# garymm/starflate

Measured on AMD Instinct MI355X. Metric: compress MiB/s + ratio vs zlib -6, 1 GiB synthetic; 1/2/4/8 GPU, higher is better.
Workload: dtype u8; 1 GPU; 1 GiB synthetic enwik-like text per GPU (gen_text_torch seed 3); effort=default, block_bytes=524288, deflate_block_bytes=32768, window_bytes=32768, container=raw, parallelism=shard1

## Files before the change

include/starflate_hip.h:

```cpp
#ifndef STARFLATE_HIP_H
#define STARFLATE_HIP_H

#include <stddef.h>
#include <stdint.h>

#ifdef __cplusplus
extern "C" {
#endif

typedef struct sfh_ctx sfh_ctx;

enum sfh_status {
  SFH_OK = 0,
  SFH_E_INVALID_ARG = -1,
  SFH_E_DST_TOO_SMALL = -2,
  SFH_E_NO_DEVICE = -3,
  SFH_E_HIP = -4,
  SFH_E_NOMEM = -5,
  SFH_E_COMM = -6,
  SFH_E_UNSUPPORTED = -7,
  SFH_E_NOT_INDEXABLE = -8
};

enum sfh_strategy {
// ... 223 lines not shown
                             uint64_t* dst_n_out, uint32_t* status);
#define SFH_STREAM_NSTAGES 5
#define SFH_STREAM_NCOUNTS 6
int sfh_last_stream_stats(sfh_ctx* ctx, float ms[SFH_STREAM_NSTAGES], uint64_t counts[SFH_STREAM_NCOUNTS]);

size_t sfh_last_decode_scratch_bytes(const sfh_ctx* ctx);

#define SFH_INFLATE_NSTAGES 2
int sfh_last_inflate_ms(sfh_ctx* ctx, float ms[SFH_INFLATE_NSTAGES]);
const char* sfh_inflate_stage_name(int stage);


int sfh_checksum_device(sfh_ctx* ctx, const void* d_src, size_t n, uint32_t kind, uint32_t* out, void* stream);
uint32_t sfh_crc32_combine(uint32_t crc_a, uint32_t crc_b, uint64_t len_b);
uint32_t sfh_adler32_combine(uint32_t adler_a, uint32_t adler_b, uint64_t len_b);

#define SFH_NSTAGES 5

void sfh_set_profiling(sfh_ctx* ctx, int on);
int sfh_last_stage_ms(sfh_ctx* ctx, float ms[SFH_NSTAGES]);
const char* sfh_stage_name(int stage);

enum sfh_debug_what {
  SFH_DBG_NTOK = 0,
  SFH_DBG_TOKENS = 1,
  SFH_DBG_ITEMS = 8,
  SFH_DBG_NITEMS = 9,
  SFH_DBG_HIST = 2,
  SFH_DBG_PLAN = 3,
  SFH_DBG_LENS = 4,
  SFH_DBG_OFFSETS = 5,
  SFH_DBG_SUBINDEX = 7,
  SFH_DBG_SEGINFO = 10,
  SFH_DBG_STAMPS = 6
};
int sfh_debug_read(sfh_ctx* ctx, int what, void* host_dst, size_t bytes);

#ifdef __cplusplus
}
#endif
#endif
```

starflate_amd/_capi.py:

```python
import ctypes as C
import os

from . import build as _build

NSTAGES = 5
INFLATE_NSTAGES = 2
SEGMENT_BYTES = 32768
STRATEGY = {"auto": 0, "stored": 1, "fixed": 2, "dynamic": 3}
CONTAINER = {"raw": 0, "zlib": 1, "gzip": 2}
COMPRESS_CONTAINER = dict(CONTAINER, dictzip=3)
DZ_MAX_CHUNKS = 32762
E_NOT_INDEXABLE = -8
SIZE_FROM_TRAILER = (1 << 64) - 1
ITEM_NOT_INDEXABLE = 0xFFFFFFF8
DBG_NTOK, DBG_TOKENS, DBG_HIST, DBG_PLAN, DBG_LENS, DBG_OFFSETS, DBG_STAMPS = range(7)
DBG_SUBINDEX = 7
DBG_ITEMS, DBG_NITEMS = 8, 9
DBG_SEGINFO = 10
DEFAULT_BLOCK_BYTES = 262144
LARGE_BLOCK_BYTES = 1 << 19
CHAIN_BLOCK_BYTES = 1 << 20
SUBINDEX_WORDS = 64

EXPORTS = [
    "sfh_default_options", "sfh_device_count", "sfh_get_device_props", "sfh_create", "sfh_destroy", "sfh_last_error",
    "sfh_compress_bound", "sfh_compress_bound_container", "sfh_dz_header_bytes", "sfh_compress", "sfh_compress_multi", "sfh_compress_device", "sfh_compress_device_async",
    "sfh_compress_batch_device_async", "sfh_compress_batch", "sfh_batch_index_size", "sfh_copy_batch_index",
    "sfh_decompress_batch_device_async", "sfh_decompress_batch",
    "sfh_decompress_ranges_device_async", "sfh_decompress_range_device", "sfh_decompress_ranges",
    "sfh_dz_read_index", "sfh_dz_read_index_device", "sfh_decompress_dz_device", "sfh_decompress_dz", "sfh_decompress_dz_ranges",
    "sfh_bgzf_bound", "sfh_compress_bgzf_device_async", "sfh_compress_bgzf_device", "sfh_compress_bgzf",
    "sfh_bgzf_read_index", "sfh_bgzf_read_index_device", "sfh_decompress_bgzf_device", "sfh_decompress_bgzf",
    "sfh_decompress_bgzf_wide_device",
    "sfh_decompress_bgzf_ranges_device", "sfh_decompress_bgzf_ranges", "sfh_bgzf_voffsets_to_offsets", "sfh_bgzf_offsets_to_voffsets",
    "sfh_zip_read_index", "sfh_zip_read_index_device", "sfh_decompress_zip_device", "sfh_decompress_zip", "sfh_zip_bound",
    "sfh_compress_zip_device_async", "sfh_compress_zip_device", "sfh_compress_zip",
    "sfh_recover_index_device", "sfh_recover_index", "sfh_decompress_any_device", "sfh_decompress_any", "sfh_last_recover_stats",
    "sfh_recover_index_batch_device", "sfh_recover_index_batch", "sfh_decompress_any_batch_device", "sfh_decompress_any_batch",
    "sfh_inflate_stream_device", "sfh_inflate_stream", "sfh_inflate_stream_batch_device", "sfh_inflate_stream_batch",
    "sfh_last_stream_stats",
    "sfh_last_block_bytes", "sfh_index_entries", "sfh_copy_index", "sfh_copy_subindex", "sfh_decompress_device", "sfh_decompress", "sfh_last_inflate_ms", "sfh_last_decode_scratch_bytes",
    "sfh_inflate_stage_name", "sfh_checksum_device", "sfh_crc32_combine", "sfh_adler32_combine",
    "sfh_set_profiling", "sfh_last_stage_ms", "sfh_stage_name", "sfh_debug_read",
    "sfh_gather_offsets", "sfh_gather_streams", "sfh_comm_ranks", "sfh_lds_order_check",
]


class Options(C.Structure):
    _fields_ = [("strategy", C.c_uint32), ("final_stream", C.c_uint32), ("lazy", C.c_uint32),
                ("no_stored_fast_path", C.c_uint32), ("container", C.c_uint32), ("block_bytes", C.c_uint32),
                ("effort", C.c_uint32), ("chain_depth", C.c_uint32)]
# ... 267 lines not shown
```

starflate_amd/compressor.py:

```python
import ctypes as C

import numpy as np

from . import _capi

CHUNK_BYTES = 32768
ITEM_NOT_INDEXABLE = _capi.ITEM_NOT_INDEXABLE


class StarflateError(RuntimeError):
    def __init__(self, code, msg):
        super().__init__(f"starflate_hip error {code}: {msg}")
        self.code = code


class Compressor:

    def __init__(self, device=0):
        self._lib = _capi.lib()
        n = self._lib.sfh_device_count()
        if n <= 0:
            raise StarflateError(-3, "no HIP device visible; the compressor has no CPU fallback")
        h = C.c_void_p()
        rc = self._lib.sfh_create(C.byref(h), int(device))
# ... 818 lines not shown

        if not (isinstance(t, torch.Tensor) and t.is_cuda and t.dtype == torch.uint8 and t.dim() == 1 and t.is_contiguous()):
            raise ValueError("expected a contiguous 1-D uint8 CUDA tensor")
        if t.device.index != self.device:
            raise ValueError(f"tensor is on cuda:{t.device.index}, compressor on cuda:{self.device}")

    def lds_order_check(self, op, blocks=256, iters=50):
        bad, n = C.c_uint64(0), C.c_uint64(0)
        rc = self._lib.sfh_lds_order_check(self._h, int(op), int(blocks), int(iters), C.byref(bad), C.byref(n))
        if rc:
            raise StarflateError(rc, self._lib.sfh_last_error(self._h).decode())
        return bad.value, n.value

    def set_profiling(self, on=True):
        self._lib.sfh_set_profiling(self._h, int(bool(on)))

    def stage_ms(self):
        ms = (C.c_float * _capi.NSTAGES)()
        self._check(self._lib.sfh_last_stage_ms(self._h, C.byref(ms)))
        return {self._lib.sfh_stage_name(k).decode(): float(ms[k]) for k in range(_capi.NSTAGES)}

    def debug(self, what, nchunks):
        shapes = {
            _capi.DBG_NTOK: ((nchunks,), np.uint32),
            _capi.DBG_TOKENS: ((nchunks, CHUNK_BYTES), np.uint32),
            _capi.DBG_HIST: ((nchunks, 576), np.uint32),
            _capi.DBG_PLAN: ((nchunks, 4), np.uint32),
            _capi.DBG_LENS: ((nchunks, 320), np.uint8),
            _capi.DBG_OFFSETS: ((nchunks,), np.uint64),
            _capi.DBG_STAMPS: ((2, nchunks, 8), np.uint64),
            _capi.DBG_SUBINDEX: ((nchunks, 32, 2), np.uint32),
            _capi.DBG_ITEMS: ((nchunks, CHUNK_BYTES), np.uint16),
            _capi.DBG_NITEMS: ((nchunks,), np.uint32),
            _capi.DBG_SEGINFO: ((nchunks, 6), np.uint32),
        }
        shape, dt = shapes[what]
        a = np.empty(shape, dtype=dt)
        self._check(self._lib.sfh_debug_read(self._h, what, a.ctypes.data, a.nbytes))
        return a

    def debug_tokens(self, nchunks):
        items = self.debug(_capi.DBG_ITEMS, nchunks)
        nit = self.debug(_capi.DBG_NITEMS, nchunks)
        toks, flags = [], []
        for c in range(nchunks):
            if nit[c] & 0x80000000:
                raise StarflateError(-1, f"chunk {c} took the stored fast path: its items are not materialised (stored_fast_path=False shows them)")
            it = items[c, : nit[c]].astype(np.uint32)
            start = (it & 0x8000) != 0
            head = start & ((it & 0x0100) != 0)
            assert not np.any(head[:-1] & start[1:]) and (it.size == 0 or not head[-1]), "a head without its distance"
            nxt = np.zeros(it.size, dtype=np.uint32)
            nxt[:-1] = it[1:]
            tok = np.where(head, np.uint32(0x80000000) | ((it & 0xFF) << 16) | (nxt & 0x7FFF), it & 0xFF)[start]
            fl = ((it & 0x4000) != 0)[start]
            reg = ((it >> 9) & 31)[start]
            toks.append(tok.astype(np.uint32))
            flags.append([(int(k), int(reg[k])) for k in np.flatnonzero(fl)])
        return toks, flags


def compress_multi(compressors, data, strategy="auto", final_stream=True, lazy=True, stored_fast_path=True, container="raw",
                   block_bytes=0):
    L = _capi.lib()
    src = np.frombuffer(data, dtype=np.uint8) if not isinstance(data, np.ndarray) else np.ascontiguousarray(data, dtype=np.uint8)
    cap = L.sfh_compress_bound(src.size, 0)
# ... 417 lines not shown
```

starflate_amd/csrc/sf_capi.hip:

```cpp
#include "../../include/starflate_hip.h"
#include "sf_any_plan.h"
#include "sf_bgzf_plan.h"
#include "sf_bgzf_range_plan.h"
#include "sf_device.h"
#include "sf_dz_plan.h"
#include "sf_inflate_core.h"
#include "sf_inflate_plan.h"
#include "sf_range_plan.h"
#include "sf_scratch.h"
#include "sf_stage_plan.h"
#include "sf_zip_plan.h"

#include <dlfcn.h>
#include <stdio.h>
#include <stdlib.h>
#include <string.h>
#include <algorithm>
#include <memory>
#include <new>
#include <thread>
#include <vector>

namespace {
using sf::scratch::Buf;
// ... 3444 lines not shown
int sfh_last_stage_ms(sfh_ctx* ctx, float ms[SFH_NSTAGES]) {
  if (!ctx || !ms || !ctx->ev_valid) return SFH_E_INVALID_ARG;
  for (int k = 0; k < SFH_NSTAGES; ++k) ms[k] = 0.f;
  for (uint32_t b = 0; b < ctx->ev_batches; ++b) {
    const Event* e = &ctx->ev[(size_t)b * sfh_ctx::kEvPerBatch];
    for (int k = 0; k < 4; ++k) {
      float t = 0.f;
      SF_HIP(hipEventElapsedTime(&t, e[k], e[k + 1]), "elapsed");
      ms[k] += t;
    }
  }
  const size_t last = (size_t)ctx->ev_batches * sfh_ctx::kEvPerBatch;
  SF_HIP(hipEventElapsedTime(&ms[4], ctx->ev[last - 1], ctx->ev[last]), "elapsed");
  return SFH_OK;
}

const char* sfh_stage_name(int stage) {
  static const char* names[SFH_NSTAGES] = {"k_lz77", "k_plan", "k_scan", "k_emit", "k_checksum"};
  return (stage >= 0 && stage < SFH_NSTAGES) ? names[stage] : "";
}

int sfh_debug_read(sfh_ctx* ctx, int what, void* host_dst, size_t bytes) {
  if (!ctx || !host_dst || !ctx->last_chunks) return SFH_E_INVALID_ARG;
  const size_t nlast = std::min<size_t>(ctx->last_chunks, std::max<uint32_t>(ctx->batch_chunks, sf::kMaxStrip / sf::kChunk));
  const size_t nc = std::min<size_t>(nlast, ctx->cap_batch), nidx = std::min<size_t>(ctx->last_chunks, ctx->cap_chunks);
  if (int rc = wait_idle(ctx)) return rc;
  const void* p = nullptr;
  size_t avail = 0;
  switch (what) {
    case SFH_DBG_NTOK: p = ctx->ws.ntok; avail = nc * 4; break;
    case SFH_DBG_TOKENS: p = ctx->ws.tokens; avail = ctx->cap_dtok >= nlast ? nlast * sf::kChunk * 4 : 0; break;
    case SFH_DBG_ITEMS: p = ctx->ws.items; avail = nc * sf::kChunk * 2; break;
    case SFH_DBG_NITEMS: p = ctx->ws.nitems; avail = nc * 4; break;
    case SFH_DBG_HIST: p = ctx->ws.hist; avail = nc * sf::kHistStride * 4; break;
    case SFH_DBG_PLAN: p = ctx->ws.plan; avail = nc * sizeof(sf::ChunkPlan); break;
    case SFH_DBG_OFFSETS: p = ctx->ws.offsets; avail = nidx * 8; break;
    case SFH_DBG_SUBINDEX: p = ctx->ws.subidx; avail = nidx * SFH_SUBINDEX_WORDS * 4; break;
    case SFH_DBG_STAMPS: p = ctx->ws.stamps; avail = p ? nc * 128 : 0; break;
    case SFH_DBG_SEGINFO: p = ctx->ws.seginfo; avail = std::min<size_t>(ctx->last_chunks * sizeof(sf::SegInfo), ctx->seginfo_cap); break;
    case SFH_DBG_LENS: {
      if (!ctx->ws.codes || bytes > nc * 320) return SFH_E_INVALID_ARG;
      SF_HIP(hipSetDevice(ctx->device), "hipSetDevice");
      SF_HIP(hipMemcpy2D(host_dst, 320, (const uint8_t*)ctx->ws.codes + offsetof(sf::ChunkCodes, lens),
                         sizeof(sf::ChunkCodes), 320, bytes / 320, hipMemcpyDeviceToHost), "debug copy");
      return SFH_OK;
    }
    default: return SFH_E_INVALID_ARG;
  }
  if (!p || bytes > avail) return SFH_E_INVALID_ARG;
  SF_HIP(hipSetDevice(ctx->device), "hipSetDevice");
  SF_HIP(hipMemcpy(host_dst, p, bytes, hipMemcpyDeviceToHost), "debug copy");
  return SFH_OK;
}

}
```

starflate_amd/csrc/sf_device.h:

```cpp
#pragma once
#include <hip/hip_runtime.h>
#include <stdint.h>

#include <vector>

#include "sf_stream_chain.h"

namespace sf {

constexpr uint32_t kChunk = 32768;
constexpr uint32_t kWindow = 32768;
constexpr uint32_t kWideRow = 65536;
constexpr uint32_t kStep = 1024;
constexpr uint32_t kHashBits = 13;
constexpr uint32_t kMaxStrip = 1u << 24;
constexpr uint32_t kRegion = 512;
constexpr uint32_t kSubBytes = 1024;
constexpr uint32_t kCap = 16;
constexpr uint32_t kMinMatch = 4;
constexpr uint32_t kFar4 = 4096;
constexpr uint32_t kSkipSlack = 128;
constexpr uint32_t kSkipProbe = 2048;
constexpr uint32_t kItemsSkipped = 0x80000000u;
constexpr uint32_t kSubRegions = kChunk / kSubBytes;
constexpr uint32_t kTokMatch = 0x80000000u;
constexpr uint32_t kTokRegion = 0x40000000u;
constexpr uint32_t kItemTok = 0x8000u;
constexpr uint32_t kItemRegion = 0x4000u;
constexpr uint32_t kItemRegionShift = 9;
constexpr uint32_t kItemHead = 0x0100u;

constexpr uint32_t kChecksumAdler32 = 1;
constexpr uint32_t kChecksumCrc32 = 2;
constexpr uint32_t kCrcPoly = 0xEDB88320u;

constexpr uint32_t kHistStride = 576;
constexpr uint32_t kHistD = 288;
constexpr uint32_t kHistLen = 320;
constexpr uint32_t kHeaderWords = 152;

template <int CTRL, int ROW_MASK>
__device__ __forceinline__ uint32_t dpp_from(uint32_t v) {
  return (uint32_t)__builtin_amdgcn_update_dpp(0, (int)v, CTRL, ROW_MASK, 0xF, false);
}
template <int CTRL, int ROW_MASK>
__device__ __forceinline__ uint32_t dpp_add_from(uint32_t v) {
  return v + (uint32_t)__builtin_amdgcn_update_dpp(0, (int)v, CTRL, ROW_MASK, 0xF, false);
}
__device__ __forceinline__ uint32_t wave_incl_add(uint32_t v) {
  v = dpp_add_from<0x111, 0xF>(v);
  v = dpp_add_from<0x112, 0xF>(v);
  v = dpp_add_from<0x114, 0xF>(v);
  v = dpp_add_from<0x118, 0xF>(v);
  v = dpp_add_from<0x142, 0xA>(v);
  v = dpp_add_from<0x143, 0xC>(v);
  return v;
}
__device__ __forceinline__ uint32_t wave_excl_max(uint32_t v) {
  v = max(v, dpp_from<0x111, 0xF>(v));
  v = max(v, dpp_from<0x112, 0xF>(v));
  v = max(v, dpp_from<0x114, 0xF>(v));
  v = max(v, dpp_from<0x118, 0xF>(v));
  v = max(v, dpp_from<0x142, 0xA>(v));
// ... 364 lines not shown
```

starflate_amd/csrc/sf_kernels.hip:

```cpp
#include "sf_device.h"

#include <stdlib.h>

namespace sf {

__device__ __forceinline__ uint32_t len_symbol(uint32_t l3, uint32_t& ebits, uint32_t& eval) {
  if (l3 == 255) { ebits = 0; eval = 0; return 285; }
  if (l3 < 8) { ebits = 0; eval = 0; return 257 + l3; }
  const uint32_t e = (31 - __builtin_clz(l3)) - 2;
  ebits = e;
  eval = l3 & ((1u << e) - 1);
  return 257 + 4 * e + 4 + ((l3 >> e) & 3);
}
__device__ __forceinline__ uint32_t dist_symbol(uint32_t d1, uint32_t& ebits, uint32_t& eval) {
  if (d1 < 4) { ebits = 0; eval = 0; return d1; }
  const uint32_t hb = 31 - __builtin_clz(d1);
  const uint32_t e = hb - 1;
  ebits = e;
  eval = d1 & ((1u << e) - 1);
  return 2 * hb + ((d1 >> e) & 1);
}
__device__ __forceinline__ uint32_t dist_symbol_of(uint32_t d1) {
  const uint32_t x = d1 > 2u ? d1 : 2u;
  const uint32_t hb = 31 - __builtin_clz(x);
// ... 920 lines not shown
            else walk(ne);
          }
        }
      }
      stamp(3);
      static_assert(kWindow == 4 * kRound && 8 * K1_THREADS == kRound && kLook % 8 == 0, "shift: four pieces per thread and the look-ahead");
      [[maybe_unused]] uint2 sh_0 = make_uint2(0, 0), sh_1 = sh_0, sh_2 = sh_0, B_early = sh_0;
      if constexpr (EARLY) {
        asm volatile("" ::: "memory");
        const uint2* s2 = reinterpret_cast<const uint2*>(smem + L_DATA);
        sh_0 = s2[kRound / 8 + t];
        sh_1 = s2[2 * kRound / 8 + t];
        sh_2 = s2[3 * kRound / 8 + t];
        B_early = s2[kWindow / 8 + t];
      }
      const uint32_t cm = marks & T;
      const uint32_t mine = (uint32_t)__popc(marks) | ((uint32_t)__popc(cm) << 16);
      const uint32_t incl = wave_incl_add(mine);
      if (lane == 63) s_wtot[wave] = incl;
      if constexpr (EARLY)
        asm volatile("" : "+v"(sh_0.x), "+v"(sh_0.y), "+v"(sh_1.x), "+v"(sh_1.y), "+v"(sh_2.x), "+v"(sh_2.y),
                          "+v"(B_early.x), "+v"(B_early.y));
      __syncthreads();
      uint32_t wbase, rtotal;
      {
        const uint32_t w = lane < K1_WAVES ? s_wtot[lane] : 0u;
        const uint32_t wi = wave_incl_add(w);
        rtotal = (uint32_t)__builtin_amdgcn_readlane((int)wi, K1_WAVES - 1);
        wbase = (uint32_t)__builtin_amdgcn_readlane((int)(wi - w), (int)wave);
      }
      static_assert(kSkipSpan == kRound, "the probe span is the chunk's first round");
      const bool skip_now = rc == 0 && fast_skip && (n - cstart) > kSkipSpan && (rtotal & 0xFFFFu) >= kSkipSpan - kSkipSlack;
      if (!skip_now && (wave & (kSubBytes / kRegion - 1)) == 0 && lane == 0)
        rtok_out[chunk * kSubRegions + rc * kRSubs + wave / (kSubBytes / kRegion)] = tot_tok + (wbase & 0xFFFFu);
      stamp(4);
      __builtin_amdgcn_s_setprio(0);

      if constexpr (EARLY) {
        if (!skip_now && r + 1 < nrounds) {
          uint2* s2 = reinterpret_cast<uint2*>(smem + L_DATA);
          s2[t] = sh_0;
          s2[kRound / 8 + t] = sh_1;
          s2[2 * kRound / 8 + t] = sh_2;
          s2[3 * kRound / 8 + t] = B_early;
          if (t >= K1_THREADS - kLook / 8) s2[kWindow / 8 + t - (K1_THREADS - kLook / 8)] = s2[(kWindow + kRound) / 8 + t - (K1_THREADS - kLook / 8)];
          *reinterpret_cast<uint2*>(&s_data[(kWindow + kLook) / 4 + 2 * t]) = make_uint2(pre_lo, pre_hi);
          age(rb + kRound);
          staged = true;
        }
      }
      if (__builtin_expect(skip_now, 0)) {
        const uint32_t clen = (n - cstart) < kChunk ? (n - cstart) : kChunk;
        const uint2 B = EARLY ? B_early : *reinterpret_cast<const uint2*>(&s_bytes[kWindow + 8 * t]);
        bool pstore = false;
        if (clen == kChunk) {
          static_assert(256 * 32 * 4 <= kWindow && kWindow / 16 == 2 * K1_THREADS, "the copies fill the window");
          static_assert(kRoundsPerChunk == 4, "the fast path's loads");
          uint4* const z4 = reinterpret_cast<uint4*>(smem + L_DATA);
          z4[t] = make_uint4(0, 0, 0, 0);
          z4[K1_THREADS + t] = make_uint4(0, 0, 0, 0);
          __syncthreads();
          uint32_t* const rep = s_data + (lane & 31u);
          auto count8 = [&](uint32_t lo, uint32_t hi) {
#pragma unroll
            for (uint32_t j = 0; j < 8; ++j) atomicAdd(&rep[(((j < 4 ? lo : hi) >> (8 * (j & 3))) & 0xFFu) * 32u], 1u);
          };
          auto fold = [&]() -> uint32_t {
// ... 10 lines not shown
            uint32_t e = ((t & 3u) == 0 && f) ? f * (est_log2(kSkipSpan) - est_log2(f)) : 0u;
            e = wave_sum(e);
            if (lane == 0) s_wtot[wave] = e;
            __syncthreads();
            const uint32_t ent = (uint32_t)__builtin_amdgcn_readfirstlane((int)wave_sum(lane < K1_WAVES ? s_wtot[lane] : 0u));
            pstore = ((ent >> 8) + 7) / 8 + kStoreMargin >= kSkipSpan;
          }
          if (!pstore) {
            uint2 w[kRoundsPerChunk - 1];
            w[0] = make_uint2(pre_lo, pre_hi);
            w[1] = *reinterpret_cast<const uint2*>(sp + cstart + 2 * kRound + kLook + 8 * t);
            w[2] = make_uint2(0, 0);
            const bool tail = 8 * t + kLook < kRound;
            if (tail) w[2] = *reinterpret_cast<const uint2*>(sp + cstart + 3 * kRound + kLook + 8 * t);
            const uint32_t look = t < kLook / 4 ? s_data[(kWindow + kRound) / 4 + t] : 0u;
            count8(w[0].x, w[0].y);
            count8(w[1].x, w[1].y);
            if (tail) count8(w[2].x, w[2].y);
            if (t < kLook / 4) {
#pragma unroll
              for (uint32_t j = 0; j < 4; ++j) atomicAdd(&rep[((look >> (8 * j)) & 0xFFu) * 32u], 1u);
            }
            __syncthreads();
            const uint32_t sum = fold();
            if ((t & 3u) == 0) s_hist[t >> 2] = sum;
          }
        } else {
#pragma unroll
          for (uint32_t k = 0; k < 8; ++k) atomicAdd(&s_hist[((k < 4 ? B.x : B.y) >> (8 * (k & 3))) & 0xFFu], 1u);
          for (uint32_t pos = cstart + kRound + t; pos < cstart + clen; pos += K1_THREADS) atomicAdd(&s_hist[sp[pos]], 1u);
        }
        const uint32_t r_last = (r + kRoundsPerChunk - 1 < nrounds ? r + kRoundsPerChunk - 1 : nrounds - 1);
        const uint32_t ctok = pstore ? 0u : clen;
        if (t < kSubRegions) rtok_out[chunk * kSubRegions + t] = t * kSubBytes < ctok ? t * kSubBytes : ctok;
        skip = true;
        lds_stale = true;
        stale_span = short_probe ? kSkipProbe : kSkipSpan;
        chunk_done = true;
        tot_tok = ctok;
        tot_items = ctok;
        rtotal = 0;
        r = r_last;
      } else
      if (marks) {
        const uint32_t before = wbase + incl - mine;
        const uint32_t ib0 = 2u * (tot_items + (before & 0xFFFFu) + (before >> 16));
        const uint32_t both = marks | (cm << 8);
        auto item_at = [&](uint32_t below) { return ib0 + 2u * (uint32_t)__popc(both & (below | (below << 8))); };
        const uint2 B = EARLY ? B_early : *reinterpret_cast<const uint2*>(&s_bytes[kWindow + pb]);
        uint32_t t_now = t;
        asm volatile("" : "+v"(t_now));
        const uint32_t flag = (t_now & (kSubBytes / 8 - 1)) == 0 ? (kItemRegion | ((rc * kRSubs + (8 * t_now) / kSubBytes) << kItemRegionShift)) : 0u;
        auto put_item = [&](uint32_t byte_off, uint32_t v) {
          *reinterpret_cast<uint16_t*>(reinterpret_cast<uint8_t*>(gi) + (uint64_t)byte_off) = (uint16_t)v;
        };
        const uint32_t lits = marks & ~cm;
#pragma unroll
        for (uint32_t k = 0; k < 8; ++k) {
          if ((lits >> k) & 1) {
            const uint32_t b = ((k < 4 ? B.x : B.y) >> (8 * (k & 3))) & 0xFFu;
            put_item(item_at((1u << k) - 1u), k == 0 ? (kItemTok | b | flag) : (kItemTok | b));
            atomicAdd(&s_hist[b], 1u);
          }
        }
        static_assert(kMinMatch >= 4, "at most two matches start in eight positions");
        uint32_t rest = cm;
#pragma unroll
        for (uint32_t it = 0; it < 2; ++it) {
          if (rest) {
            const uint32_t k = (uint32_t)__builtin_ctz(rest);
            rest &= rest - 1u;
            const uint32_t at = item_at((1u << k) - 1u);
            uint32_t l3 = (N >> (4 * k)) & 15u;
            uint32_t d1 = dm1_of(k);
            if (l3 == kCap - 3) {
              l3 = cap_len - 3;
              d1 = cap_run ? 0u : d1;
            }
            put_item(at, (kItemTok | kItemHead | l3) | (k == 0 ? flag : 0u));
            put_item(at + 2, d1);
            atomicAdd(&s_hist[kHistLen + l3], 1u);
            atomicAdd(&s_hist[kHistD + smem[LD + (d1 < 256 ? d1 : 256 + (d1 >> 7))]], 1u);
          }
        }
      }
      tot_tok += rtotal & 0xFFFFu;
      tot_items += (rtotal & 0xFFFFu) + (rtotal >> 16);
      if constexpr (STAMPS) __syncthreads();
      stamp(5);
    }

    if (chunk_done || rc == kRoundsPerChunk - 1 || r + 1 == nrounds) {
      __syncthreads();
      if (!(chunk_done && tot_tok == 0))
        for (uint32_t idx = t; idx < kHistStride; idx += K1_THREADS) {
          hist_out[(uint64_t)chunk * kHistStride + idx] = s_hist[idx];
          s_hist[idx] = (idx == 256) ? 1u : 0u;
        }
      if (t == 0) { ntok_out[chunk] = tot_tok; nitems_out[chunk] = tot_items | (skip ? kItemsSkipped : 0u); }
      const uint32_t covered = chunk_done ? kSubRegions : (rc + 1) * kRSubs;
      if (t < kSubRegions && t >= covered) rtok_out[chunk * kSubRegions + t] = tot_tok;
      stamp(6);
    }
  }
  if (nrounds == 0) {
    for (uint32_t idx = t; idx < kHistStride; idx += K1_THREADS) hist_out[(uint64_t)chunk0 * kHistStride + idx] = (idx == 256) ? 1u : 0u;
    if (t == 0) { ntok_out[chunk0] = 0; nitems_out[chunk0] = 0; }
    if (t < kSubRegions) rtok_out[chunk0 * kSubRegions + t] = 0;
  }
  if constexpr (STAMPS) {
    if (t == 0)
      for (int k = 0; k < 8; ++k) stamps[(uint64_t)strip * 8 + k] = st_acc[k];
  }
}


__device__ __forceinline__ void or_bits(uint32_t* stage, uint32_t bitpos, uint64_t value) {
  const uint32_t w = bitpos >> 5, sh = bitpos & 31;
  const uint64_t v0 = value << sh;
  const uint32_t v2 = sh ? (uint32_t)(value >> (64 - sh)) : 0u;
  const uint32_t lo = (uint32_t)v0, mid = (uint32_t)(v0 >> 32);
  if (lo) atomicOr(&stage[w], lo);
  if (mid) atomicOr(&stage[w + 1], mid);
  if (v2) atomicOr(&stage[w + 2], v2);
}

struct PlanSmem {
  uint32_t freq[320];
  uint32_t key[288];
  union {
    uint16_t w[576];
    struct { uint16_t w_head[64]; uint8_t rle_sym[320]; uint8_t rle_ext[320]; };
  };
  union {
// ... 630 lines not shown
  if (t == 0) {
    const uint64_t all = base + s_tile[K3_TILES];
    if constexpr (!BATCH) *total = all;
    offsets[nchunks] = all + lead;
  }
  if constexpr (BATCH) {
    __syncthreads();
    for (uint32_t i = t; i < nitems; i += K3_THREADS) {
      BatchItem& I = bitems[i];
      const uint64_t g0 = offsets[I.chunk0], g1 = offsets[I.chunk0 + I.nchunks];
      const uint64_t start = I.carry ? total[I.out] : hdr;
      I.shift = start - g0;
      total[I.out] = start + (g1 - g0);
    }
  }
}

constexpr uint32_t K4_THREADS = 512;
constexpr uint32_t K4_WAVES = K4_THREADS / 64;
constexpr uint32_t K4_IPT = 8;
constexpr uint32_t K4_STAGE_FORCED = 9392;
constexpr uint32_t K4_STAGE_AUTO = 8200;
static_assert(4 * K4_STAGE_FORCED >= 3 + kChunk + kChunk / 8 + 640 + 16 + 8, "k_emit: the stage holds the largest chunk");
static_assert(4 * K4_STAGE_AUTO >= 3 + kChunk + kStoredExtra - 1 + 16 + 8, "k_emit: the small stage holds the largest chunk "
              "plan_chunk codes under strategy 0");
static_assert(K4_STAGE_FORCED % 4 == 0 && K4_STAGE_AUTO % 4 == 0, "the stage is zeroed in 16-byte steps");
template <uint32_t STAGE_WORDS>
struct EmitLds {
  alignas(16) uint32_t stage[STAGE_WORDS];
  uint32_t lcode[288];
  uint32_t dcode[32];
  uint32_t tab[1024];
  uint32_t wtot[2][K4_WAVES];
  uint32_t rtok[kSubRegions];
};
template <uint32_t STAGE_WORDS>
constexpr uint32_t k4_waves_per_simd() { return STAGE_WORDS == K4_STAGE_AUTO ? 8 : 6; }
static_assert(k4_waves_per_simd<K4_STAGE_AUTO>() / 2 * sizeof(EmitLds<K4_STAGE_AUTO>) <= 160 * 1024, "k_emit: four workgroups per CU");
static_assert(k4_waves_per_simd<K4_STAGE_FORCED>() / 2 * sizeof(EmitLds<K4_STAGE_FORCED>) <= 160 * 1024, "k_emit: three workgroups per CU");

typedef uint16_t u16x2 __attribute__((ext_vector_type(2)));
typedef int16_t s16x2 __attribute__((ext_vector_type(2)));

__device__ __forceinline__ void literal_bits(uint32_t byte, const uint32_t* lcode, uint64_t& value, uint32_t& nb) {
  const uint32_t lc = lcode[byte];
  value = lc & 0xFFFF;
  nb = lc >> 16;
}
__device__ __forceinline__ uint32_t lenlut_entry(uint32_t l3, const uint32_t* lcode) {
  uint32_t le, lv;
  const uint32_t lc = lcode[len_symbol(l3, le, lv)];
  const uint32_t p = lc >> 16;
  return (lc & 0xFFFFu) | (lv << p) | ((p + le) << 24);
}
__device__ __forceinline__ void match_bits(uint32_t l3, uint32_t d1, const uint32_t* lenlut, const uint32_t* dcode,
                                           uint64_t& value, uint32_t& nb) {
  uint32_t de, dv;
  const uint32_t ds = dist_symbol(d1, de, dv);
  const uint32_t le = lenlut[l3], dc = dcode[ds];
  uint32_t p = le >> 24;
  uint64_t v = le & 0xFFFFFFu;
  v |= (uint64_t)(dc & 0xFFFF) << p;
  p += dc >> 16;
  v |= (uint64_t)dv << p;
  p += de;
  value = v;
  nb = p;
}

template <bool BATCH, uint32_t STAGE_WORDS>
__global__ __launch_bounds__(K4_THREADS, k4_waves_per_simd<STAGE_WORDS>()) void k_emit(const uint8_t* __restrict__ src, uint64_t n_total,
                                                     uint32_t , uint16_t* items,
                                                     const uint32_t* __restrict__ nitems_in,
                                                     const uint32_t* __restrict__ ntok_in,
                                                     const ChunkPlan* __restrict__ plan,
                                                     const ChunkCodes* __restrict__ codes,
                                                     const uint64_t* __restrict__ offsets,
                                                     const uint32_t* __restrict__ rtok,
                                                     uint32_t* __restrict__ subidx,
                                                     uint8_t* __restrict__ dst_all,
                                                     const BatchChunk* __restrict__ bchunks,
                                                     const BatchItem* __restrict__ bitems) {
  __shared__ EmitLds<STAGE_WORDS> L;
  uint32_t(&s_stage)[STAGE_WORDS] = L.stage;
  uint32_t(&s_lcode)[288] = L.lcode;
  uint32_t(&s_dcode)[32] = L.dcode;
  uint32_t(&s_tab)[1024] = L.tab;
  uint32_t(&s_wtot)[2][K4_WAVES] = L.wtot;
  uint32_t(&s_rtok)[kSubRegions] = L.rtok;
  static_assert(K4_THREADS == 512, "one table entry per thread and kind");
  constexpr uint32_t kTabLit = 512, kTabLen = 768, kTabDistN = 510;

  const uint32_t t = threadIdx.x, lane = t & 63;
  const uint32_t wave = (uint32_t)__builtin_amdgcn_readfirstlane((int)(t >> 6));
  const uint32_t chunk = blockIdx.x;
  const ChunkPlan P = plan[chunk];
  const uint8_t* csrc;
  uint8_t* dst;
  uint64_t off = offsets[chunk];
  uint32_t n_raw;
  if constexpr (BATCH) {
    const BatchChunk B = bchunks[chunk];
    const BatchItem& I = bitems[B.item >> 1];
    csrc = B.src;
    n_raw = B.n_raw;
    dst = I.dst;
    off += I.shift;
  } else {
    const uint64_t cbase = (uint64_t)chunk * kChunk;
    csrc = src + cbase;
    n_raw = (uint32_t)((n_total - cbase) < (uint64_t)kChunk ? (n_total - cbase) : kChunk);
    dst = dst_all;
  }
  const ChunkCodes& C = codes[chunk];
  uint32_t pre_code = t < 288 ? C.lcode[t] : (t < 320 ? C.dcode[t - 288] : 0u);
  uint32_t pre_rtok = t < kSubRegions ? rtok[(uint64_t)chunk * kSubRegions + t] : 0u;
  const uint32_t pre_ntok = ntok_in[chunk], pre_nit = nitems_in[chunk];
  asm volatile("" : "+v"(pre_code), "+v"(pre_rtok));

  uint32_t* const sub = subidx + (uint64_t)chunk * 2 * kSubRegions;
  if (P.btype == 0) {
    if (t < 2 * kSubRegions) sub[t] = 0;
// ... 38 lines not shown
    }
    const uint32_t head = (uint32_t)((4 - ((uintptr_t)d & 3)) & 3);
    const uint32_t h = head < n_raw ? head : n_raw;
    if (t < h) d[t] = sp[t];
    const uint32_t nd = (n_raw - h) / 4;
    uint32_t* d32 = reinterpret_cast<uint32_t*>(d + h);
    const uint32_t* s32 = reinterpret_cast<const uint32_t*>(sp);
    const uint32_t full_src_words = n_raw / 4;
    for (uint32_t k = t; k < nd; k += K4_THREADS) {
      const uint32_t ob = h + 4 * k;
      const uint32_t w = ob >> 2;
      uint32_t lo = s32[w], hi = 0;
      if ((ob & 3) != 0) {
        if (w + 1 < full_src_words) hi = s32[w + 1];
        else
          for (uint32_t b = 0; b < 4 && 4 * (w + 1) + b < n_raw; ++b) hi |= (uint32_t)sp[4 * (w + 1) + b] << (8 * b);
      }
      d32[k] = __builtin_amdgcn_alignbyte(hi, lo, ob & 3);
    }
    const uint32_t done = h + 4 * nd;
    if (t < n_raw - done) d[done + t] = sp[done + t];
    return;
  }

  const uint32_t sh = (uint32_t)(off & 3);
  const uint32_t nwords = (sh + P.out_bytes + 3) / 4;
  {
    uint4* z = reinterpret_cast<uint4*>(s_stage);
    for (uint32_t k = t; k < (nwords + 2 + 3) / 4 && k < STAGE_WORDS / 4; k += K4_THREADS) z[k] = make_uint4(0, 0, 0, 0);
  }
  if (t < 288) s_lcode[t] = pre_code;
  else if (t < 320) s_dcode[t - 288] = pre_code;
  if (t < kSubRegions) {
    s_rtok[t] = pre_rtok;
    sub[2 * t + 1] = pre_rtok;
  }
  __syncthreads();
  if (t < 256) {
    const uint32_t le = lenlut_entry(t, s_lcode);
    s_tab[kTabLen + t] = (le & 0xFFFFFu) | (le >> 24) * (1u << 20 | 1u << 27);
    s_tab[kTabLit + t] = (pre_code & 0xFFFFu) | (pre_code >> 16) * (1u << 20 | 1u << 27);
  }
  if (t < kTabDistN) {
    const uint32_t sym = dist_symbol_of(t < 256 ? t : (t - 254) << 7);
    const uint32_t dc = s_dcode[sym];
    s_tab[t] = (dc & 0xFFFFu) | ((dc >> 16) << 20) | (((dc >> 16) + dist_extra_of_sym(sym)) << 27);
  } else {
    s_tab[t] = 0;
  }
  {
    uint8_t* sb = reinterpret_cast<uint8_t*>(s_stage) + sh;
    const uint8_t* hb = reinterpret_cast<const uint8_t*>(C.header);
    const uint32_t hbytes = (P.header_bits + 7) / 8;
    for (uint32_t k = t; k < hbytes; k += K4_THREADS) sb[k] = hb[k];
  }
  __syncthreads();

  const uint32_t ntok = pre_ntok;
  const uint32_t nit = pre_nit & ~kItemsSkipped;
  const uint16_t* it = items + (uint64_t)chunk * kChunk;
  if (pre_nit & kItemsSkipped) {
    uint16_t* const wr = items + (uint64_t)chunk * kChunk;
    for (uint32_t pos = t; pos < nit; pos += K4_THREADS) {
      const uint32_t b = csrc[pos];
      wr[pos] = (uint16_t)(kItemTok | ((pos & (kSubBytes - 1)) == 0 ? (b | kItemRegion | ((pos / kSubBytes) << kItemRegionShift)) : b));
    }
    __threadfence_block();
    __syncthreads();
  }
  uint32_t running = 8 * sh + P.header_bits;
  uint32_t buf = 0;
  uint4 q_next = make_uint4(0, 0, 0, 0);
  if (nit) q_next = *reinterpret_cast<const uint4*>(it + t * K4_IPT);
  for (uint32_t b0 = 0; b0 < nit; b0 += K4_THREADS * K4_IPT, buf ^= 1) {
    const uint32_t i0 = b0 + t * K4_IPT;
    const uint4 q = q_next;
    const bool full = b0 + K4_THREADS * K4_IPT <= nit;
    if (b0 + K4_THREADS * K4_IPT < nit) q_next = *reinterpret_cast<const uint4*>(it + i0 + K4_THREADS * K4_IPT);
    const uint32_t qd[K4_IPT / 2] = {q.x, q.y, q.z, q.w};
    uint32_t val[K4_IPT], nb[K4_IPT], mine = 0;
    uint32_t ent[K4_IPT];
#pragma unroll
    for (uint32_t j = 0; j < K4_IPT / 2; ++j) {
      static_assert(kItemHead == 0x100 && kTabLen == kTabLit + 0x100 && kTabLit == 0x200, "a token's low nine bits are its table index");
      static_assert(kItemTok == 0x8000, "bit 15 tells a token's first item from a distance");
      const u16x2 w = __builtin_bit_cast(u16x2, qd[j]);
      const uint32_t itok = (qd[j] & 0x01FF01FFu) | (kTabLit * 0x10001u);
      const u16x2 idist = __builtin_elementwise_min(w, (u16x2)(w >> (uint16_t)7) + (uint16_t)254);
      uint32_t tok = __builtin_bit_cast(uint32_t, __builtin_bit_cast(s16x2, w) >> (int16_t)15);
      asm volatile("" : "+v"(tok));
      const uint32_t idx = (tok & itok) | (~tok & __builtin_bit_cast(uint32_t, idist));
      const uint32_t by = __builtin_bit_cast(uint32_t, (u16x2)(__builtin_bit_cast(u16x2, idx) << (uint16_t)2));
      ent[2 * j] = *reinterpret_cast<const uint32_t*>(reinterpret_cast<const uint8_t*>(s_tab) + (by & 0xFFFFu));
      ent[2 * j + 1] = *reinterpret_cast<const uint32_t*>(reinterpret_cast<const uint8_t*>(s_tab) + (by >> 16));
    }
    asm volatile("" : "+v"(ent[0]), "+v"(ent[1]), "+v"(ent[2]), "+v"(ent[3]), "+v"(ent[4]), "+v"(ent[5]), "+v"(ent[6]), "+v"(ent[7]));
    auto both = [](uint32_t w) { return w & (w << 1) & 0x80008000u; };
    auto sbit = [](uint32_t k) { return (k & 1) ? 15 + k : k; };
    uint32_t starts = (both(q.x) >> 15) | (both(q.y) >> 13) | (both(q.z) >> 11) | (both(q.w) >> 9);
    if (!full) {
      uint32_t left = nit - i0;
      left = i0 < nit ? left : 0u;
#pragma unroll
      for (uint32_t k = 0; k < K4_IPT; ++k) {
        ent[k] = k < left ? ent[k] : 0u;
        starts &= k < left ? ~0u : ~(1u << sbit(k));
      }
    }
    const uint32_t s0 = starts ? (uint32_t)__builtin_ctz(starts) : 32u;
    const bool walk = __ballot((starts & (starts - 1)) != 0) != 0;
    uint32_t off0 = 0;
#pragma unroll
    for (uint32_t k = 0; k < K4_IPT; ++k) {
      const uint32_t en = ent[k];
      const uint32_t dl = en >> 20, n = en >> 27;
      val[k] = (__builtin_amdgcn_ubfe(qd[k / 2], 16 * (k & 1), (n - dl) & 31u) << (dl & 31u)) | (en & 0xFFFFFu);
      nb[k] = n;
      asm volatile("" : "+v"(val[k]), "+v"(nb[k]));
      off0 = s0 == sbit(k) ? mine : off0;
      mine += nb[k];
    }
    uint32_t region0;
    {
      const uint32_t j = (s0 >> 1) & 3u;
      const uint32_t w = j == 0 ? q.x : j == 1 ? q.y : j == 2 ? q.z : q.w;
      region0 = (w >> ((s0 & 16u) + kItemRegionShift)) & 31u;
    }
    const uint32_t incl = wave_incl_add(mine);
    if (lane == 63) s_wtot[buf][wave] = incl;
    __syncthreads();
    uint32_t pre = 0, all = 0;
#pragma unroll
    for (uint32_t w = 0; w < K4_WAVES; ++w) {
      const uint32_t v = s_wtot[buf][w];
      if (w < wave) pre += v;
      all += v;
    }
    const uint32_t pos = running + pre + incl - mine;
    if (walk) {
      const uint4 r = *reinterpret_cast<const uint4*>(it + i0);
      const uint32_t rd[K4_IPT / 2] = {r.x, r.y, r.z, r.w};
      uint32_t pk = pos;
#pragma unroll
      for (uint32_t k = 0; k < K4_IPT; ++k) {
        const uint32_t e = (rd[k / 2] >> (16 * (k & 1))) & 0xFFFFu;
        if ((e & (kItemTok | kItemRegion)) == (kItemTok | kItemRegion) && i0 + k < nit)
          sub[2 * ((e >> kItemRegionShift) & 31u)] = pk - 8 * sh;
        pk += nb[k];
      }
    } else if (starts) {
      sub[2 * region0] = pos + off0 - 8 * sh;
    }
    uint32_t wi = pos >> 5, ab = pos & 31;
    uint64_t acc = 0;
    auto put = [&](uint32_t v32, uint32_t n) {
      acc |= (uint64_t)v32 << ab;
      ab += n;
      if (ab >= 32) {
        atomicOr(&s_stage[wi++], (uint32_t)acc);
        acc >>= 32;
        ab -= 32;
      }
    };
#pragma unroll
    for (uint32_t k = 0; k < K4_IPT; ++k) put(val[k], nb[k]);
    if (ab) atomicOr(&s_stage[wi], (uint32_t)acc);
    running += all;
  }
  __syncthreads();
  if (t < kSubRegions && s_rtok[t] >= ntok) sub[2 * t] = running - 8 * sh;
  if (t == 0) {
    const uint32_t eob = s_lcode[256];
    or_bits(s_stage, running, eob & 0xFFFF);
    const uint32_t endbit = running + (eob >> 16);
    if (!(C.header[0] & 1u)) {
      const uint32_t byte = (endbit + 3 + 7) / 8;
      or_bits(s_stage, 8 * (byte + 2), 0xFFFFull);
    }
  }
  __syncthreads();

  uint8_t* gbase = dst + (off - sh);
  uint32_t* g32 = reinterpret_cast<uint32_t*>(gbase);
  const uint32_t lo_b = sh, hi_b = sh + P.out_bytes;
  for (uint32_t w = t; w < nwords; w += K4_THREADS) {
    const uint32_t v = s_stage[w];
    if (4 * w >= lo_b && 4 * w + 4 <= hi_b) {
      g32[w] = v;
    } else {
#pragma unroll
      for (uint32_t b = 0; b < 4; ++b) {
        const uint32_t idx = 4 * w + b;
        if (idx >= lo_b && idx < hi_b) gbase[idx] = (uint8_t)(v >> (8 * b));
      }
    }
  }
}

hipError_t init_kernels() { return hipSuccess; }

hipError_t launch_lz77(const uint8_t* src, uint64_t n, uint32_t nchunks, const Workspace& ws,
                       const Options& opt, hipStream_t s, const BatchTables* bt) {
  if (opt.strip_bytes == 0 || opt.strip_bytes % kChunk || opt.strip_bytes > kMaxStrip) return hipErrorInvalidValue;
// ... 80 lines not shown
```

Baseline: 238,800 MiB/s.

## Record per-region item index in rtok to locate subindex starts in encoder

```diff
diff --git a/include/starflate_hip.h b/include/starflate_hip.h
--- a/include/starflate_hip.h
+++ b/include/starflate_hip.h
@@ -279,6 +279,7 @@
   SFH_DBG_OFFSETS = 5,
   SFH_DBG_SUBINDEX = 7,
   SFH_DBG_SEGINFO = 10,
+  SFH_DBG_RITEM = 11,
   SFH_DBG_STAMPS = 6
 };
 int sfh_debug_read(sfh_ctx* ctx, int what, void* host_dst, size_t bytes);
diff --git a/starflate_amd/_capi.py b/starflate_amd/_capi.py
--- a/starflate_amd/_capi.py
+++ b/starflate_amd/_capi.py
@@ -17,6 +17,7 @@
 DBG_SUBINDEX = 7
 DBG_ITEMS, DBG_NITEMS = 8, 9
 DBG_SEGINFO = 10
+DBG_RITEM = 11
 DEFAULT_BLOCK_BYTES = 262144
 LARGE_BLOCK_BYTES = 1 << 19
 CHAIN_BLOCK_BYTES = 1 << 20
diff --git a/starflate_amd/compressor.py b/starflate_amd/compressor.py
--- a/starflate_amd/compressor.py
+++ b/starflate_amd/compressor.py
@@ -874,6 +874,7 @@
             _capi.DBG_SUBINDEX: ((nchunks, 32, 2), np.uint32),
             _capi.DBG_ITEMS: ((nchunks, CHUNK_BYTES), np.uint16),
             _capi.DBG_NITEMS: ((nchunks,), np.uint32),
+            _capi.DBG_RITEM: ((nchunks, 32), np.uint32),
             _capi.DBG_SEGINFO: ((nchunks, 6), np.uint32),
         }
         shape, dt = shapes[what]
diff --git a/starflate_amd/csrc/sf_capi.hip b/starflate_amd/csrc/sf_capi.hip
--- a/starflate_amd/csrc/sf_capi.hip
+++ b/starflate_amd/csrc/sf_capi.hip
@@ -3500,6 +3500,13 @@
     case SFH_DBG_TOKENS: p = ctx->ws.tokens; avail = ctx->cap_dtok >= nlast ? nlast * sf::kChunk * 4 : 0; break;
     case SFH_DBG_ITEMS: p = ctx->ws.items; avail = nc * sf::kChunk * 2; break;
     case SFH_DBG_NITEMS: p = ctx->ws.nitems; avail = nc * 4; break;
+    case SFH_DBG_RITEM: {
+      if (!ctx->ws.rtok || bytes % 4 || bytes > nc * sf::kSubRegions * 4) return SFH_E_INVALID_ARG;
+      SF_HIP(hipSetDevice(ctx->device), "hipSetDevice");
+      SF_HIP(hipMemcpy(host_dst, ctx->ws.rtok, bytes, hipMemcpyDeviceToHost), "debug copy");
+      for (size_t k = 0; k < bytes / 4; ++k) static_cast<uint32_t*>(host_dst)[k] >>= 16;
+      return SFH_OK;
+    }
     case SFH_DBG_HIST: p = ctx->ws.hist; avail = nc * sf::kHistStride * 4; break;
     case SFH_DBG_PLAN: p = ctx->ws.plan; avail = nc * sizeof(sf::ChunkPlan); break;
     case SFH_DBG_OFFSETS: p = ctx->ws.offsets; avail = nidx * 8; break;
diff --git a/starflate_amd/csrc/sf_device.h b/starflate_amd/csrc/sf_device.h
--- a/starflate_amd/csrc/sf_device.h
+++ b/starflate_amd/csrc/sf_device.h
@@ -29,6 +29,8 @@
 constexpr uint32_t kItemRegion = 0x4000u;
 constexpr uint32_t kItemRegionShift = 9;
 constexpr uint32_t kItemHead = 0x0100u;
+static_assert(kChunk <= 0x8000u, "a chunk's token and item counts fit 16 bits each");
+constexpr uint32_t region_word(uint32_t tokens_before, uint32_t items_before) { return tokens_before | (items_before << 16); }
 
 constexpr uint32_t kChecksumAdler32 = 1;
 constexpr uint32_t kChecksumCrc32 = 2;
diff --git a/starflate_amd/csrc/sf_kernels.hip b/starflate_amd/csrc/sf_kernels.hip
--- a/starflate_amd/csrc/sf_kernels.hip
+++ b/starflate_amd/csrc/sf_kernels.hip
@@ -976,7 +976,8 @@
       static_assert(kSkipSpan == kRound, "the probe span is the chunk's first round");
       const bool skip_now = rc == 0 && fast_skip && (n - cstart) > kSkipSpan && (rtotal & 0xFFFFu) >= kSkipSpan - kSkipSlack;
       if (!skip_now && (wave & (kSubBytes / kRegion - 1)) == 0 && lane == 0)
-        rtok_out[chunk * kSubRegions + rc * kRSubs + wave / (kSubBytes / kRegion)] = tot_tok + (wbase & 0xFFFFu);
+        rtok_out[chunk * kSubRegions + rc * kRSubs + wave / (kSubBytes / kRegion)] =
+            region_word(tot_tok + (wbase & 0xFFFFu), tot_items + (wbase & 0xFFFFu) + (wbase >> 16));
       stamp(4);
       __builtin_amdgcn_s_setprio(0);
 
@@ -1053,7 +1054,10 @@
         }
         const uint32_t r_last = (r + kRoundsPerChunk - 1 < nrounds ? r + kRoundsPerChunk - 1 : nrounds - 1);
         const uint32_t ctok = pstore ? 0u : clen;
-        if (t < kSubRegions) rtok_out[chunk * kSubRegions + t] = t * kSubBytes < ctok ? t * kSubBytes : ctok;
+        if (t < kSubRegions) {
+          const uint32_t before = t * kSubBytes < ctok ? t * kSubBytes : ctok;
+          rtok_out[chunk * kSubRegions + t] = region_word(before, before);
+        }
         skip = true;
         lds_stale = true;
         stale_span = short_probe ? kSkipProbe : kSkipSpan;
@@ -1120,7 +1124,7 @@
         }
       if (t == 0) { ntok_out[chunk] = tot_tok; nitems_out[chunk] = tot_items | (skip ? kItemsSkipped : 0u); }
       const uint32_t covered = chunk_done ? kSubRegions : (rc + 1) * kRSubs;
-      if (t < kSubRegions && t >= covered) rtok_out[chunk * kSubRegions + t] = tot_tok;
+      if (t < kSubRegions && t >= covered) rtok_out[chunk * kSubRegions + t] = region_word(tot_tok, tot_items);
       stamp(6);
     }
   }
@@ -1817,7 +1821,7 @@
   uint32_t dcode[32];
   uint32_t tab[1024];
   uint32_t wtot[2][K4_WAVES];
-  uint32_t rtok[kSubRegions];
+  uint32_t rtab[2 * kSubRegions];
 };
 template <uint32_t STAGE_WORDS>
 constexpr uint32_t k4_waves_per_simd() { return STAGE_WORDS == K4_STAGE_AUTO ? 8 : 6; }
@@ -1872,7 +1876,7 @@
   uint32_t(&s_dcode)[32] = L.dcode;
   uint32_t(&s_tab)[1024] = L.tab;
   uint32_t(&s_wtot)[2][K4_WAVES] = L.wtot;
-  uint32_t(&s_rtok)[kSubRegions] = L.rtok;
+  uint32_t(&s_rtab)[2 * kSubRegions] = L.rtab;
   static_assert(K4_THREADS == 512, "one table entry per thread and kind");
   constexpr uint32_t kTabLit = 512, kTabLen = 768, kTabDistN = 510;
 
@@ -1977,8 +1981,9 @@
   if (t < 288) s_lcode[t] = pre_code;
   else if (t < 320) s_dcode[t - 288] = pre_code;
   if (t < kSubRegions) {
-    s_rtok[t] = pre_rtok;
-    sub[2 * t + 1] = pre_rtok;
+    s_rtab[t] = pre_rtok & 0xFFFFu;
+    s_rtab[kSubRegions + t] = pre_rtok >> 16;
+    sub[2 * t + 1] = pre_rtok & 0xFFFFu;
   }
   __syncthreads();
   if (t < 256) {
@@ -2040,21 +2045,12 @@
       ent[2 * j + 1] = *reinterpret_cast<const uint32_t*>(reinterpret_cast<const uint8_t*>(s_tab) + (by >> 16));
     }
     asm volatile("" : "+v"(ent[0]), "+v"(ent[1]), "+v"(ent[2]), "+v"(ent[3]), "+v"(ent[4]), "+v"(ent[5]), "+v"(ent[6]), "+v"(ent[7]));
-    auto both = [](uint32_t w) { return w & (w << 1) & 0x80008000u; };
-    auto sbit = [](uint32_t k) { return (k & 1) ? 15 + k : k; };
-    uint32_t starts = (both(q.x) >> 15) | (both(q.y) >> 13) | (both(q.z) >> 11) | (both(q.w) >> 9);
     if (!full) {
       uint32_t left = nit - i0;
       left = i0 < nit ? left : 0u;
 #pragma unroll
-      for (uint32_t k = 0; k < K4_IPT; ++k) {
-        ent[k] = k < left ? ent[k] : 0u;
-        starts &= k < left ? ~0u : ~(1u << sbit(k));
-      }
-    }
-    const uint32_t s0 = starts ? (uint32_t)__builtin_ctz(starts) : 32u;
-    const bool walk = __ballot((starts & (starts - 1)) != 0) != 0;
-    uint32_t off0 = 0;
+      for (uint32_t k = 0; k < K4_IPT; ++k) ent[k] = k < left ? ent[k] : 0u;
+    }
 #pragma unroll
     for (uint32_t k = 0; k < K4_IPT; ++k) {
       const uint32_t en = ent[k];
@@ -2062,14 +2058,7 @@
       val[k] = (__builtin_amdgcn_ubfe(qd[k / 2], 16 * (k & 1), (n - dl) & 31u) << (dl & 31u)) | (en & 0xFFFFFu);
       nb[k] = n;
       asm volatile("" : "+v"(val[k]), "+v"(nb[k]));
-      off0 = s0 == sbit(k) ? mine : off0;
       mine += nb[k];
-    }
-    uint32_t region0;
-    {
-      const uint32_t j = (s0 >> 1) & 3u;
-      const uint32_t w = j == 0 ? q.x : j == 1 ? q.y : j == 2 ? q.z : q.w;
-      region0 = (w >> ((s0 & 16u) + kItemRegionShift)) & 31u;
     }
     const uint32_t incl = wave_incl_add(mine);
     if (lane == 63) s_wtot[buf][wave] = incl;
@@ -2082,38 +2071,54 @@
       all += v;
     }
     const uint32_t pos = running + pre + incl - mine;
-    if (walk) {
-      const uint4 r = *reinterpret_cast<const uint4*>(it + i0);
-      const uint32_t rd[K4_IPT / 2] = {r.x, r.y, r.z, r.w};
-      uint32_t pk = pos;
-#pragma unroll
-      for (uint32_t k = 0; k < K4_IPT; ++k) {
-        const uint32_t e = (rd[k / 2] >> (16 * (k & 1))) & 0xFFFFu;
-        if ((e & (kItemTok | kItemRegion)) == (kItemTok | kItemRegion) && i0 + k < nit)
-          sub[2 * ((e >> kItemRegionShift) & 31u)] = pk - 8 * sh;
-        pk += nb[k];
-      }
-    } else if (starts) {
-      sub[2 * region0] = pos + off0 - 8 * sh;
-    }
-    uint32_t wi = pos >> 5, ab = pos & 31;
-    uint64_t acc = 0;
+    const uint32_t wi0 = b0 + wave * (64 * K4_IPT);
+    const uint32_t rit = s_rtab[kSubRegions + (lane & (kSubRegions - 1))];
+    const bool mine_due = rit - wi0 < 64 * K4_IPT && rit < nit;
+    uint32_t due = (uint32_t)__ballot(mine_due);
+    if (__builtin_popcount(due) > 2) {
+      uint32_t a = nb[0] | nb[1] << 8 | nb[2] << 16 | nb[3] << 24, b = nb[4] | nb[5] << 8 | nb[6] << 16;
+      a += a << 8;
+      a += a << 16;
+      b += b << 8;
+      b += b << 16;
+      b += (a >> 24) * 0x010101u;
+      const uint32_t at = rit - wi0, from = ((at / K4_IPT) & 63u) * 4, slot = at & (K4_IPT - 1);
+      const uint32_t pos_o = (uint32_t)__builtin_amdgcn_ds_bpermute((int)from, (int)pos);
+      const uint32_t a_o = (uint32_t)__builtin_amdgcn_ds_bpermute((int)from, (int)a);
+      const uint32_t b_o = (uint32_t)__builtin_amdgcn_ds_bpermute((int)from, (int)b);
+      const uint32_t front = slot ? ((slot < 5 ? a_o : b_o) >> (8 * ((slot - 1) & 3u))) & 0xFFu : 0u;
+      if (mine_due && lane < kSubRegions) sub[2 * lane] = pos_o + front - 8 * sh;
+      due = 0;
+    }
+    while (due) {
+      const uint32_t r = (uint32_t)__builtin_ctz(due);
+      due &= due - 1;
+      const uint32_t at = (uint32_t)__builtin_amdgcn_readlane((int)rit, (int)r) - wi0;
+      const uint32_t in_front = (1u << (at & (K4_IPT - 1))) - 1u;
+      uint32_t front = pos - 8 * sh;
+#pragma unroll
+      for (uint32_t k = 0; k + 1 < K4_IPT; ++k) front += nb[k] & (uint32_t)((int32_t)(in_front << (31 - k)) >> 31);
+      if (lane == at / K4_IPT) sub[2 * r] = front;
+    }
+    uint32_t wb = (pos >> 5) << 2, ab = pos & 31, lo = 0;
     auto put = [&](uint32_t v32, uint32_t n) {
-      acc |= (uint64_t)v32 << ab;
+      const uint64_t v = (uint64_t)v32 << ab;
+      lo |= (uint32_t)v;
       ab += n;
       if (ab >= 32) {
-        atomicOr(&s_stage[wi++], (uint32_t)acc);
-        acc >>= 32;
+        atomicOr(reinterpret_cast<uint32_t*>(reinterpret_cast<uint8_t*>(s_stage) + wb), lo);
+        lo = (uint32_t)(v >> 32);
+        wb += 4;
         ab -= 32;
       }
     };
 #pragma unroll
     for (uint32_t k = 0; k < K4_IPT; ++k) put(val[k], nb[k]);
-    if (ab) atomicOr(&s_stage[wi], (uint32_t)acc);
+    if (ab) atomicOr(reinterpret_cast<uint32_t*>(reinterpret_cast<uint8_t*>(s_stage) + wb), lo);
     running += all;
   }
   __syncthreads();
-  if (t < kSubRegions && s_rtok[t] >= ntok) sub[2 * t] = running - 8 * sh;
+  if (t < kSubRegions && s_rtab[t] >= ntok) sub[2 * t] = running - 8 * sh;
   if (t == 0) {
     const uint32_t eob = s_lcode[256];
     or_bits(s_stage, running, eob & 0xFFFF);
```

Result: faster. 241,300 MiB/s (median of 6 runs) (+1.0%).
